# Safari77/rupphash

Hardware: AMD Instinct MI355X
Metric: pdq_hashes_per_sec_512x512_rgb (higher is better)
Workload: dtype f32

## Files before the change

### rupphash_amd/csrc/pdq_fused512.hip

```cpp
#include "pdq_tail.hpp"
#include "rph_internal.h"

namespace {

typedef _Float16 h2 __attribute__((ext_vector_type(2)));
typedef _Float16 h8 __attribute__((ext_vector_type(8)));

template <int SW_, int CH_ = 3, bool PARK_ = true>
struct Geo {
    static constexpr int SW = SW_;
    static constexpr int CH = CH_;
    static constexpr int NSTRIP = 512 / SW;
    static constexpr int CL = SW / 8;
    static constexpr int NG = 64 / CL;
    static constexpr int NH = 64 / (NG * 8);
    static constexpr int NOCT = SW / 8;
    static constexpr int TILE_PITCH = SW * 2 + 16;
    static constexpr int TILE_BYTES = 64 * TILE_PITCH;
    static constexpr int OFF_TILE = 0;
    static constexpr int OFF_XCHG = NH == 2 ? 32 * TILE_PITCH : 0;
    static constexpr int OFF_STATE = TILE_BYTES;
    static constexpr int OFF_EDGE = OFF_STATE + 7168;
#ifndef RPH_PARK_CHAINS
#define RPH_PARK_CHAINS 1
#endif
    static constexpr bool PARK = RPH_PARK_CHAINS && PARK_ && SW == 64;
    static constexpr int OFF_PARK_C = OFF_EDGE + 1536;
    static constexpr int OFF_PARK_E = OFF_PARK_C + (PARK ? 9 * 64 * 4 : 0);
    static constexpr int LDS_BYTES = OFF_PARK_E + (PARK ? 9 * 6 * 4 : 0);
    static constexpr int WAVES_PER_SIMD = 2;
    static constexpr bool AHEAD = SW == 64;
    static_assert(64 * 33 * 4 <= TILE_BYTES, "sample transpose buffer must fit in the dead V tile");
    static_assert((NG - 1) * 7 * CL * 16 <= (NH == 2 ? 32 : 64) * TILE_PITCH, "exchange area must fit");
    static_assert(rph::TAIL_LDS_FLOATS * 4 <= TILE_BYTES, "tail scratch must fit in the dead V tile");
};
constexpr int SAMP_PITCH = 33;

struct Px8 {
    uint32_t d[6];
};
struct __attribute__((packed, aligned(4))) U3 {
    uint32_t x, y, z;
};

struct __attribute__((packed, aligned(4))) U2 {
    uint32_t x, y;
};
template <int CH = 3>
__device__ __forceinline__ Px8 load_px8(const uint8_t *p)
{
    Px8 r;
    if (CH == 1) {
        const U2 a = *reinterpret_cast<const U2 *>(p);
        r.d[0] = a.x; r.d[1] = a.y; r.d[2] = r.d[3] = r.d[4] = r.d[5] = 0;
        return r;
    }
    const U3 a = *reinterpret_cast<const U3 *>(p);
    const U3 b = *reinterpret_cast<const U3 *>(p + 12);
    r.d[0] = a.x; r.d[1] = a.y; r.d[2] = a.z; r.d[3] = b.x; r.d[4] = b.y; r.d[5] = b.z;
    return r;
}

template <int P>
__device__ __forceinline__ float luma_px(const Px8 &v)
{
    constexpr int B = 3 * P;
    const float r = (float)((v.d[B >> 2] >> (8 * (B & 3))) & 0xFFu);
    const float g = (float)((v.d[(B + 1) >> 2] >> (8 * ((B + 1) & 3))) & 0xFFu);
    const float b = (float)((v.d[(B + 2) >> 2] >> (8 * ((B + 2) & 3))) & 0xFFu);
    const float num = __builtin_fmaf(299.0f, r, __builtin_fmaf(587.0f, g, __builtin_fmaf(114.0f, b, 500.0f)));
    return __builtin_truncf(num * 0.001f);
}

template <int CH = 3>
__device__ __forceinline__ void luma8(const Px8 &v, float (&l)[8])
{
    if (CH == 1) {
#pragma unroll
        for (int i = 0; i < 8; i++) l[i] = (float)((v.d[i >> 2] >> (8 * (i & 3))) & 0xFFu);
        return;
    }
    l[0] = luma_px<0>(v); l[1] = luma_px<1>(v); l[2] = luma_px<2>(v); l[3] = luma_px<3>(v);
    l[4] = luma_px<4>(v); l[5] = luma_px<5>(v); l[6] = luma_px<6>(v); l[7] = luma_px<7>(v);
}

constexpr uint32_t BIASED_ZERO = 0x64006400u;
struct Row8 {
    h2 q[4];
};
__device__ __forceinline__ h2 h2_bits(uint32_t u) { return __builtin_bit_cast(h2, u); }
__device__ __forceinline__ h2 byte_pair_lo(uint32_t d) { return h2_bits(__builtin_amdgcn_perm(0x64646464u, d, 0x04010400u)); }
__device__ __forceinline__ h2 byte_pair_hi(uint32_t d) { return h2_bits(__builtin_amdgcn_perm(0x64646464u, d, 0x04030402u)); }

__device__ __forceinline__ float dot2_from_zero(h2 a, h2 k, uint32_t after)
{
    float r;
    asm volatile("v_dot2_f32_f16 %0, %1, %2, 0" : "=v"(r) : "v"(__builtin_bit_cast(uint32_t, a)), "s"(__builtin_bit_cast(uint32_t, k)), "v"(after));
    return r;
}

struct Pairs12 {
    h2 P[12];
};
__device__ __forceinline__ Pairs12 byte_pairs(const Px8 &v)
{
    Pairs12 r;
#pragma unroll
    for (int i = 0; i < 6; i++) {
        r.P[2 * i] = byte_pair_lo(v.d[i]);
        r.P[2 * i + 1] = byte_pair_hi(v.d[i]);
    }
    return r;
}
__device__ __forceinline__ Row8 luma_row(const Pairs12 &pr, bool zero, uint32_t &order)
{
    const h2 *P = pr.P;
    const h2 k_rg = h2{(_Float16)299.0f, (_Float16)587.0f};
    const h2 k_b0 = h2{(_Float16)114.0f, (_Float16)0.0f};
    const h2 k_0r = h2{(_Float16)0.0f, (_Float16)299.0f};
    const h2 k_gb = h2{(_Float16)587.0f, (_Float16)114.0f};
    float vhalf;
    asm("v_mov_b32 %0, 0.5" : "=v"(vhalf));
    h2 packed[4];
#pragma unroll
    for (int pp = 0; pp < 4; pp++) {
        const float n0 = __builtin_amdgcn_fdot2(P[3 * pp], k_rg, dot2_from_zero(P[3 * pp + 1], k_b0, order), false);
        const float n1 = __builtin_amdgcn_fdot2(P[3 * pp + 1], k_0r, dot2_from_zero(P[3 * pp + 2], k_gb, order), false);
        const float y0 = __builtin_fmaf(n0, 0.001f, vhalf), y1 = __builtin_fmaf(n1, 0.001f, vhalf);
        packed[pp] = __builtin_bit_cast(h2, __builtin_amdgcn_cvt_pkrtz(y0, y1));
    }
    order = __builtin_bit_cast(uint32_t, packed[3]);
    Row8 r;
#pragma unroll
    for (int i = 0; i < 4; i++) {
        r.q[i] = packed[i];
        if (zero) r.q[i] = h2_bits(BIASED_ZERO);
    }
    return r;
}
__device__ __forceinline__ Row8 luma_row_gray(const Px8 &v, bool zero, uint32_t &order)
{
    Row8 r;
    r.q[0] = byte_pair_lo(v.d[0]);
    r.q[1] = byte_pair_hi(v.d[0]);
    r.q[2] = byte_pair_lo(v.d[1]);
    r.q[3] = byte_pair_hi(v.d[1]);
#pragma unroll
    for (int i = 0; i < 4; i++)
        if (zero) r.q[i] = h2_bits(BIASED_ZERO);
    order = __builtin_bit_cast(uint32_t, r.q[3]);
    return r;
}
template <int CH = 3>
__device__ __forceinline__ Row8 pack_row(const Px8 &v, bool zero, uint32_t &order)
{
    if (CH == 1) return luma_row_gray(v, zero, order);
    return luma_row(byte_pairs(v), zero, order);
}
__device__ __forceinline__ uint4 row_bits(const Row8 &r)
{
    uint4 u;
    u.x = __builtin_bit_cast(uint32_t, r.q[0]);
    u.y = __builtin_bit_cast(uint32_t, r.q[1]);
    u.z = __builtin_bit_cast(uint32_t, r.q[2]);
    u.w = __builtin_bit_cast(uint32_t, r.q[3]);
    return u;
}
__device__ __forceinline__ Row8 bits_row(const uint4 &u)
{
    Row8 r;
    r.q[0] = __builtin_bit_cast(h2, u.x);
    r.q[1] = __builtin_bit_cast(h2, u.y);
    r.q[2] = __builtin_bit_cast(h2, u.z);
    r.q[3] = __builtin_bit_cast(h2, u.w);
    return r;
}

__device__ __forceinline__ float div_small(float N, float d, float dinv)
{
    const float q0 = N * dinv;
    const float r = __builtin_fmaf(-q0, d, N);
    return __builtin_fmaf(r, dinv, q0);
}

__device__ __forceinline__ void wave_lds_fence() { asm volatile("" ::: "memory"); }

struct Wave {
    uint8_t *lds;
    const uint8_t *img;
    size_t row_stride;
    uint32_t rs32;
    int lane;
    float hs, sum, ring[8];
    uint4 pv;
    float row_d8, row_dinv8;
    float smp[32];
    float smp_last;
    float csum, cring[8];
    float ecs, ering[8];
    float bnew[8];
    rph::TailAcc tail;
    bool want_quality;
};

template <class G>
__device__ __forceinline__ int half_row(int b, int h, int g, int k) { return 64 * b + 4 + (G::NG * 8) * h + 8 * g + k; }

template <class G>
__device__ __forceinline__ void half_offsets(const Wave &w, int b, int s, int h, uint32_t &off0, uint32_t &off_max)
{
    const int c = w.lane & (G::CL - 1), g = w.lane / G::CL;
    const uint32_t col = (uint32_t)(G::SW * s + 8 * c) * (uint32_t)G::CH;
    off0 = (uint32_t)half_row<G>(b, h, g, 0) * w.rs32 + col;
    off_max = 511u * w.rs32 + col;
}
template <int CH>
__device__ __forceinline__ Px8 load_px8_at(const Wave &w, uint32_t off) { return load_px8<CH>(w.img + off); }

template <class G>
__device__ __forceinline__ void half_issue(const Wave &w, int b, int s, int h, Px8 (&pre)[8])
{
    uint32_t off, off_max;
    half_offsets<G>(w, b, s, h, off, off_max);
#pragma unroll
    for (int k = 0; k < 8; k++) {
        pre[k] = load_px8_at<G::CH>(w, off);
        off = off + w.rs32;
        off = off < off_max ? off : off_max;
    }
}

template <class G, bool LAST_BAND>
__device__ __forceinline__ void half_luma(const Wave &w, int b, int h, Px8 (&pre)[8], Row8 (&L)[8], bool has_next, int nb, int ns, int nh)
{
    const int g = w.lane / G::CL;
    uint32_t off, off_max;
    half_offsets<G>(w, nb, ns, nh, off, off_max);
    uint32_t order = 0;
#pragma unroll
    for (int k = 0; k < 8; k++) {
        if (G::CH == 1) {
            const Px8 cur = pre[k];
            if (has_next) pre[k] = load_px8_at<1>(w, off);
            off = off + w.rs32;
            off = off < off_max ? off : off_max;
            L[k] = luma_row_gray(cur, LAST_BAND && (half_row<G>(b, h, g, k) >= 512), order);
            continue;
        }
        const Pairs12 pr = byte_pairs(pre[k]);
        if (has_next) pre[k] = load_px8_at<3>(w, off);
        off = off + w.rs32;
        off = off < off_max ? off : off_max;
        L[k] = luma_row(pr, LAST_BAND && (half_row<G>(b, h, g, k) >= 512), order);
    }
}

template <class G>
__device__ __forceinline__ void half_build(Wave &w, int s, int h, const Row8 (&L)[8])
{
    const int c = w.lane & (G::CL - 1), g = w.lane / G::CL;
    uint8_t *tile = w.lds + G::OFF_TILE;
    uint8_t *xchg = w.lds + G::OFF_XCHG;
    uint8_t *state = w.lds + G::OFF_STATE + (G::SW * s + 8 * c) * 2;

    if (g < G::NG - 1) {
        uint8_t *x = xchg + ((g * 7) * G::CL + c) * 16;
#pragma unroll
        for (int k = 1; k < 8; k++) *reinterpret_cast<uint4 *>(x + (k - 1) * (G::CL * 16)) = row_bits(L[k]);
    }
    wave_lds_fence();
    Row8 hist[7];
    {
        const uint8_t *hp = (g == 0) ? state : xchg + (((g - 1) * 7) * G::CL + c) * 16;
        const int stride = (g == 0) ? 1024 : G::CL * 16;
#pragma unroll
        for (int j = 0; j < 7; j++) hist[j] = bits_row(*reinterpret_cast<const uint4 *>(hp + j * stride));
    }
    wave_lds_fence();
    if (g == G::NG - 1) {
#pragma unroll
        for (int k = 1; k < 8; k++) *reinterpret_cast<uint4 *>(state + (k - 1) * 1024) = row_bits(L[k]);
    }
    const int row0 = (G::NG * 8) * h + 8 * g;
    Row8 v;
#pragma unroll
    for (int i = 0; i < 4; i++) {
        const h2 two_bias = h2{(_Float16)2048.0f, (_Float16)2048.0f};
        h2 a = hist[0].q[i] + (hist[1].q[i] - two_bias);
        h2 bb = hist[2].q[i] + (hist[3].q[i] - two_bias);
        h2 cc = hist[4].q[i] + (hist[5].q[i] - two_bias);
        h2 dd = hist[6].q[i] + (L[0].q[i] - two_bias);
        v.q[i] = (a + bb) + (cc + dd);
    }
    *reinterpret_cast<uint4 *>(tile + (row0 + 0) * G::TILE_PITCH + 16 * c) = row_bits(v);
#pragma unroll
    for (int m = 1; m < 8; m++) {
#pragma unroll
        for (int i = 0; i < 4; i++) v.q[i] = (v.q[i] - hist[m - 1].q[i]) + L[m].q[i];
        *reinterpret_cast<uint4 *>(tile + (row0 + m) * G::TILE_PITCH + 16 * c) = row_bits(v);
    }
    wave_lds_fence();
}

__device__ __forceinline__ uint32_t h2_diff(uint32_t cur, uint32_t prev)
{
    return __builtin_bit_cast(uint32_t, __builtin_bit_cast(h2, cur) - __builtin_bit_cast(h2, prev));
}
template <int HI>
__device__ __forceinline__ float hs_step(float hs, uint32_t packed)
{
    float r;
    if (HI)
        asm("v_fma_mix_f32 %0, %1, 1.0, %2 op_sel:[1,0,0] op_sel_hi:[1,0,0]" : "=v"(r) : "v"(packed), "v"(hs));
    else
        asm("v_fma_mix_f32 %0, %1, 1.0, %2 op_sel:[0,0,0] op_sel_hi:[1,0,0]" : "=v"(r) : "v"(packed), "v"(hs));
    return r;
}
template <int HI>
__device__ __forceinline__ float hs_sub(float hs, uint32_t packed)
{
    float r;
    if (HI)
        asm("v_fma_mix_f32 %0, %1, -1.0, %2 op_sel:[1,0,0] op_sel_hi:[1,0,0]" : "=v"(r) : "v"(packed), "v"(hs));
    else
        asm("v_fma_mix_f32 %0, %1, -1.0, %2 op_sel:[0,0,0] op_sel_hi:[1,0,0]" : "=v"(r) : "v"(packed), "v"(hs));
    return r;
}

template <int E>
__device__ __forceinline__ void row_step(Wave &w, float in2)
{
    constexpr int slot = (E + 4) & 7;
    w.sum = w.sum + in2;
    w.sum = w.sum - w.ring[slot];
    w.ring[slot] = in2;
}

template <bool EDGE_ROWS>
__device__ __forceinline__ float pass1_value(const Wave &w, float hs)
{
    if (EDGE_ROWS) return div_small(hs, w.row_d8, w.row_dinv8);
    return hs;
}

template <class G, bool EDGE_ROWS, bool FIRST, bool LAST>
__device__ __forceinline__ void scan_strip(Wave &w)
{
    const int r = w.lane;
    const uint8_t *tp = w.lds + G::OFF_TILE + r * G::TILE_PITCH;
    const float *edge = reinterpret_cast<const float *>(w.lds + G::OFF_EDGE);
    float fresh[G::NOCT];
#pragma unroll
    for (int q = 0; q < G::NOCT; q++) {
        const uint4 cur = *reinterpret_cast<const uint4 *>(tp + 16 * q);
        const uint32_t dq[4] = {h2_diff(cur.x, w.pv.x), h2_diff(cur.y, w.pv.y), h2_diff(cur.z, w.pv.z), h2_diff(cur.w, w.pv.w)};
        const bool first_octet = FIRST && q == 0;
        float e0 = 0.f, e1 = 0.f, e2 = 0.f;
        if (first_octet) {
            e0 = edge[0 * 64 + r];
            e1 = edge[1 * 64 + r];
            e2 = edge[2 * 64 + r];
        }
#define RPH_STEP(E)                                                              \
    {                                                                            \
        w.hs = hs_step<(E) & 1>(w.hs, dq[(E) >> 1]);                             \
        float in2 = pass1_value<EDGE_ROWS>(w, w.hs);                             \
        if (first_octet && (E) == 4) in2 = e0;                                   \
        if (first_octet && (E) == 5) in2 = e1;                                   \
        if (first_octet && (E) == 6) in2 = e2;                                   \
        if (!(first_octet && (E) < 4)) row_step<E>(w, in2);  \
    }
        RPH_STEP(0) RPH_STEP(1) RPH_STEP(2) RPH_STEP(3) RPH_STEP(4)
        fresh[q] = w.sum * 0.125f;
        RPH_STEP(5) RPH_STEP(6) RPH_STEP(7)
#undef RPH_STEP
        w.pv = cur;
    }
    if (LAST) {
        const float e3 = edge[3 * 64 + r], e4 = edge[4 * 64 + r], e5 = edge[5 * 64 + r];
        w.hs = hs_sub<0>(w.hs, w.pv.x); row_step<0>(w, e3);
        w.hs = hs_sub<1>(w.hs, w.pv.x); row_step<1>(w, e4);
        w.hs = hs_sub<0>(w.hs, w.pv.y); row_step<2>(w, e5);
        w.hs = hs_sub<1>(w.hs, w.pv.y);
        {
            const float in511 = (EDGE_ROWS ? div_small(w.hs, w.row_d8, w.row_dinv8) : w.hs) * 2.0f;
            row_step<3>(w, in511);
        }
        w.sum = w.sum - w.ring[0];
        w.smp_last = w.sum / 7.0f;
    }
#pragma unroll
    for (int i = 0; i < 32 - G::NOCT; i++) w.smp[i] = w.smp[i + G::NOCT];
#pragma unroll
    for (int q = 0; q < G::NOCT; q++) w.smp[32 - G::NOCT + q] = fresh[q];
}

__device__ __forceinline__ void scan_reset(Wave &w, int b)
{
    w.hs = 0.f;
    w.sum = 0.f;
#pragma unroll
    for (int i = 0; i < 8; i++) w.ring[i] = 0.f;
    w.pv = make_uint4(0, 0, 0, 0);
    const int y = 64 * b + w.lane;
    const int lo = y - 3 < 0 ? 0 : y - 3, hi = y + 4 > 511 ? 511 : y + 4;
    const float d = (float)(hi - lo + 1);
    w.row_d8 = d * 0.125f;
    w.row_dinv8 = (1.0f / d) * 8.0f;
}

template <class G, bool NEXT_EDGE = false>
__device__ __forceinline__ void col_pass(Wave &w, int b, bool second_half, Px8 (*epx)[2] = nullptr)
{
    float *tb = reinterpret_cast<float *>(w.lds + G::OFF_TILE);
#pragma unroll
    for (int t = 0; t < 32; t++) tb[w.lane * SAMP_PITCH + t] = w.smp[t];
    tb[w.lane * SAMP_PITCH + 32] = w.smp_last;
    if (NEXT_EDGE) edge_band_issue<G>(w, b + 1, *epx);
    wave_lds_fence();
    const bool active = second_half ? (w.lane >= 31) : (w.lane < 31);
    if (active) {
        float *park = reinterpret_cast<float *>(w.lds + G::OFF_PARK_C) + w.lane;
        if (G::PARK) {
            w.csum = park[0];
#pragma unroll
            for (int e = 0; e < 8; e++) w.cring[e] = park[64 * (e + 1)];
        }
        const float *samp = tb + (second_half ? w.lane - 31 : w.lane + 1);
#pragma unroll
        for (int u = 0; u < 8; u++) {
            float in[8];
#pragma unroll
            for (int e = 0; e < 8; e++) in[e] = samp[(8 * u + e) * SAMP_PITCH];
#pragma unroll
            for (int e = 0; e < 8; e++) {
                w.csum = w.csum + in[e];
                w.csum = w.csum - w.cring[e];
                w.cring[e] = in[e];
                if (e == 0) w.bnew[u] = w.csum * (0.125f * 0.015625f);
            }
        }
        if (G::PARK) {
            park[0] = w.csum;
#pragma unroll
            for (int e = 0; e < 8; e++) park[64 * (e + 1)] = w.cring[e];
        }
    }
    wave_lds_fence();
}

template <int CH>
__device__ __forceinline__ void edge_issue(const Wave &w, int y, Px8 (&e)[2])
{
    const int yc = y > 511 ? 511 : y;
    e[0] = load_px8<CH>(w.img + (size_t)yc * w.row_stride);
    e[1] = load_px8<CH>(w.img + (size_t)yc * w.row_stride + 504 * CH);
}
__device__ __forceinline__ void edge_values(const float (&l)[8], const float (&r)[8], bool live, float (&rv)[6])
{
    const float r0 = (((l[0] + l[1]) + l[2]) + l[3]) + l[4];
    const float r1 = r0 + l[5];
    const float r2 = r1 + l[6];
    const float q510 = (((r[3] + r[4]) + r[5]) + r[6]) + r[7];
    const float q509 = q510 + r[2];
    const float q508 = q509 + r[1];
    rv[0] = div_small(r0 * 64.0f, 5.0f, 1.0f / 5.0f);
    rv[1] = div_small(r1 * 64.0f, 6.0f, 1.0f / 6.0f);
    rv[2] = div_small(r2 * 64.0f, 7.0f, 1.0f / 7.0f);
    rv[3] = div_small(q508 * 64.0f, 7.0f, 1.0f / 7.0f);
    rv[4] = div_small(q509 * 64.0f, 6.0f, 1.0f / 6.0f);
    rv[5] = div_small(q510 * 64.0f, 5.0f, 1.0f / 5.0f);
    if (!live) {
#pragma unroll
        for (int k = 0; k < 6; k++) rv[k] = 0.f;
    }
}
template <int CH>
__device__ __forceinline__ void edge_compute(const Px8 (&e)[2], bool live, float (&rv)[6])
{
    float l[8], r[8];
    luma8<CH>(e[0], l);
    luma8<CH>(e[1], r);
    edge_values(l, r, live, rv);
}
template <int CH>
__device__ __forceinline__ void edge_rowvals(const Wave &w, int y, bool live, float (&rv)[6])
{
    Px8 e[2];
    edge_issue<CH>(w, y, e);
    edge_compute<CH>(e, live, rv);
}

template <class G>
__device__ __forceinline__ void edge_prologue(Wave &w)
{
    float *edge = reinterpret_cast<float *>(w.lds + G::OFF_EDGE);
    float rv[6];
    {
        const uint8_t *row = w.lds + G::OFF_STATE + (3 + (w.lane & 3)) * 1024;
        const h8 hl = *reinterpret_cast<const h8 *>(row), hr = *reinterpret_cast<const h8 *>(row + 504 * 2);
        float l[8], r[8];
#pragma unroll
        for (int i = 0; i < 8; i++) {
            l[i] = (float)hl[i] - 1024.0f;
            r[i] = (float)hr[i] - 1024.0f;
        }
        edge_values(l, r, true, rv);
    }
    if (w.lane < 4) {
#pragma unroll
        for (int k = 0; k < 6; k++) edge[k * 64 + w.lane] = rv[k];
    }
    wave_lds_fence();
    w.ecs = 0.f;
#pragma unroll
    for (int i = 0; i < 8; i++) w.ering[i] = 0.f;
    if (w.lane < 6) {
#pragma unroll
        for (int t = 0; t < 4; t++) {
            const float v = edge[w.lane * 64 + t];
            w.ecs = w.ecs + v;
            w.ering[t] = v;
        }
        if (G::PARK) {
            float *park = reinterpret_cast<float *>(w.lds + G::OFF_PARK_E) + w.lane;
            park[0] = w.ecs;
#pragma unroll
            for (int i = 0; i < 8; i++) park[6 * (i + 1)] = w.ering[i];
        }
    }
    wave_lds_fence();
}

template <class G>
__device__ __forceinline__ void edge_band_issue(const Wave &w, int b, Px8 (&epx)[2]) { edge_issue<G::CH>(w, 64 * b + 4 + w.lane, epx); }

template <class G, int KIND>
__device__ __forceinline__ void edge_band(Wave &w, int b, const Px8 (&epx)[2])
{
    float *edge = reinterpret_cast<float *>(w.lds + G::OFF_EDGE);
    {
        float rv[6];
        const int y = 64 * b + 4 + w.lane;
        edge_compute<G::CH>(epx, y < 512, rv);
#pragma unroll
        for (int k = 0; k < 6; k++) edge[k * 64 + w.lane] = rv[k];
    }
    wave_lds_fence();
    if (w.lane < 6) {
        float *mine = edge + w.lane * 64;
        float *park = reinterpret_cast<float *>(w.lds + G::OFF_PARK_E) + w.lane;
        if (G::PARK) {
            w.ecs = park[0];
#pragma unroll
            for (int i = 0; i < 8; i++) w.ering[i] = park[6 * (i + 1)];
        }
#pragma unroll 1
        for (int u = 0; u < 8; u++) {
            float in[8], out[8];
#pragma unroll
            for (int e = 0; e < 8; e++) in[e] = mine[8 * u + e];
#pragma unroll
            for (int e = 0; e < 8; e++) {
                constexpr int dummy = 0;
                (void)dummy;
                const int slot = (e + 4) & 7;
                const bool add = !(KIND == 2 && u == 7 && e >= 4);
                if (add) w.ecs = w.ecs + in[e];
                w.ecs = w.ecs - w.ering[slot];
                w.ering[slot] = in[e];
                float o;
                if (KIND == 0 && u == 0 && e < 3)
                    o = w.ecs / (float)(5 + e);
                else if (KIND == 2 && u == 7 && e >= 4)
                    o = w.ecs / (float)(11 - e);
                else
                    o = w.ecs * 0.125f;
                out[e] = o;
            }
#pragma unroll
            for (int e = 0; e < 8; e++) mine[8 * u + e] = out[e];
        }
        if (G::PARK) {
            park[0] = w.ecs;
#pragma unroll
            for (int i = 0; i < 8; i++) park[6 * (i + 1)] = w.ering[i];
        }
    }
    wave_lds_fence();
}

template <class G>
__device__ __forceinline__ void store_samples(const Wave &w, float *band_samples, bool second_half)
{
    float *p = band_samples + (second_half ? 32 * 64 : 0) + w.lane;
    asm volatile("" : "+v"(p));
#pragma unroll
    for (int t = 0; t < 32; t++) p[t * 64] = w.smp[t];
    if (second_half) p[32 * 64] = w.smp_last;
}

template <class G, int KIND, bool LL = false>
__device__ __forceinline__ void do_band(Wave &w, int b, Px8 (&pre)[8], float *samples, Px8 (&epx)[2])
{
    constexpr bool EDGE_ROWS = KIND != 1;
    if (!LL) {
        if (!G::AHEAD) edge_band_issue<G>(w, b, epx);
        edge_band<G, KIND>(w, b, epx);
    }
    scan_reset(w, b);
#pragma unroll 1
    for (int s = 0; s < G::NSTRIP; s++) {
#pragma unroll 1
        for (int h = 0; h < G::NH; h++) {
            Row8 L[8];
            int nb = b, ns = s, nh = h + 1;
            if (nh == G::NH) {
                nh = 0;
                ns = s + 1;
                if (ns == G::NSTRIP) {
                    ns = 0;
                    nb = b + 1;
                }
            }
            half_luma<G, KIND == 2>(w, b, h, pre, L, LL ? nb == b : nb < 8, nb, ns, nh);
            half_build<G>(w, s, h, L);
        }
        if (s == 0)
            scan_strip<G, EDGE_ROWS, true, false>(w);
        else if (s == G::NSTRIP - 1)
            scan_strip<G, EDGE_ROWS, false, true>(w);
        else
            scan_strip<G, EDGE_ROWS, false, false>(w);
        wave_lds_fence();
        if (LL) {
            if (s == G::NSTRIP / 2 - 1) store_samples<G>(w, samples, false);
            if (s == G::NSTRIP - 1) store_samples<G>(w, samples, true);
        } else {
            if (s == G::NSTRIP / 2 - 1) col_pass<G>(w, b, false);
            if (!G::AHEAD && s == G::NSTRIP - 1) col_pass<G>(w, b, true);
        }
        wave_lds_fence();
    }
    if (LL) return;
    if (G::AHEAD) {
        col_pass<G, KIND != 2>(w, b, true, &epx);
        wave_lds_fence();
    }
#pragma unroll
    for (int u = 0; u < 8; u++)
        if (KIND != 0 || u > 0) rph::tail_row(w.tail, w.bnew[u], 8 * b + u - 1, w.lane, w.want_quality);
}

template <class G>
__global__ void __launch_bounds__(64, G::WAVES_PER_SIMD) pdq_fused512_kernel(const uint8_t *__restrict__ px, uint32_t n, size_t row_stride,
                                                          size_t image_stride, uint8_t *hash, float *quality, float *coeffs,
                                                          uint8_t *dihedral, uint8_t *valid)
{
    __shared__ __attribute__((aligned(16))) uint8_t lds[G::LDS_BYTES];
    const uint32_t img = blockIdx.x;
    Wave w;
    w.lds = lds;
    w.img = px + (size_t)img * image_stride;
    w.row_stride = row_stride;
    w.rs32 = (uint32_t)row_stride;
    w.lane = threadIdx.x;
    Px8 head[4], epx[2], pre[8];
    if (G::AHEAD) {
#pragma unroll
        for (int row = 0; row < 4; row++) head[row] = load_px8<G::CH>(w.img + (size_t)row * row_stride + (size_t)(8 * w.lane) * G::CH);
        edge_band_issue<G>(w, 0, epx);
    }
    half_issue<G>(w, 0, 0, 0, pre);
    wave_lds_fence();
    w.csum = 0.f;
    w.smp_last = 0.f;
#pragma unroll
    for (int i = 0; i < 32; i++) w.smp[i] = 0.f;
#pragma unroll
    for (int i = 0; i < 8; i++) w.cring[i] = 0.f;
    if (G::PARK) {
#pragma unroll
        for (int i = 0; i < 9; i++) reinterpret_cast<float *>(lds + G::OFF_PARK_C)[64 * i + w.lane] = 0.f;
    }
    rph::tail_init(w.tail);
    w.want_quality = quality != nullptr;
#pragma unroll
    for (int u = 0; u < 8; u++) w.bnew[u] = 0.f;

    {
        for (int j = 0; j < 3; j++)
            for (int t = w.lane; t < 64; t += 64) *reinterpret_cast<uint4 *>(lds + G::OFF_STATE + j * 1024 + t * 16) = make_uint4(BIASED_ZERO, BIASED_ZERO, BIASED_ZERO, BIASED_ZERO);
        uint32_t order = 0;
        if (G::AHEAD) {
#pragma unroll
            for (int row = 0; row < 4; row++)
                *reinterpret_cast<uint4 *>(lds + G::OFF_STATE + (3 + row) * 1024 + (8 * w.lane) * 2) = row_bits(pack_row<G::CH>(head[row], false, order));
        } else {
#pragma unroll 1
            for (int it = 0; it < 4; it++) {
                const int slot = it * 64 + w.lane;
                const int chunk = slot & 63, row = slot >> 6;
                const Px8 p = load_px8<G::CH>(w.img + (size_t)row * row_stride + (size_t)(8 * chunk) * G::CH);
                *reinterpret_cast<uint4 *>(lds + G::OFF_STATE + (3 + row) * 1024 + (8 * chunk) * 2) = row_bits(pack_row<G::CH>(p, false, order));
            }
        }
    }
    wave_lds_fence();
    edge_prologue<G>(w);

    do_band<G, 0>(w, 0, pre, nullptr, epx);
#pragma unroll 1
    for (int b = 1; b < 7; b++) do_band<G, 1>(w, b, pre, nullptr, epx);
    do_band<G, 2>(w, 7, pre, nullptr, epx);

    if (G::PARK) {
        w.csum = reinterpret_cast<const float *>(lds + G::OFF_PARK_C)[w.lane];
        w.cring[0] = reinterpret_cast<const float *>(lds + G::OFF_PARK_C)[64 + w.lane];
    }
    w.csum = w.csum - w.cring[0];
    rph::tail_row(w.tail, (w.csum / 7.0f) * 0.015625f, 63, w.lane, w.want_quality);

    __syncthreads();
    rph::tail_finish(w.tail, reinterpret_cast<float *>(lds), w.lane, hash + (size_t)img * 32, quality ? quality + img : nullptr,
                  coeffs ? coeffs + (size_t)img * 256 : nullptr, dihedral ? dihedral + (size_t)img * 256 : nullptr);
    if (valid && w.lane == 0) valid[img] = 1;
}

constexpr int LL_SAMPLE_FLOATS = 8 * 65 * 64;
constexpr int LL_EDGE_PITCH = 520;

template <class G, int KIND>
__device__ __forceinline__ void ll_band(Wave &w, int b, float *samples)
{
    Px8 pre[8];
    half_issue<G>(w, b, 0, 0, pre);
    Px8 none[2];
    do_band<G, KIND, true>(w, b, pre, samples, none);
}

template <class G>
__global__ void __launch_bounds__(512, 2) pdq_fused512_ll_kernel(const uint8_t *__restrict__ px, uint32_t n, size_t row_stride, size_t image_stride,
                                                                 float *__restrict__ sample_scratch, uint8_t *hash, float *quality, float *coeffs,
                                                                 uint8_t *dihedral, uint8_t *valid)
{
    static_assert(G::NH == 1, "the low-latency kernel is built on the 64-px strip geometry");
    __shared__ __attribute__((aligned(16))) uint8_t lds[8 * G::LDS_BYTES + 6 * LL_EDGE_PITCH * 4];
    const uint32_t img = blockIdx.x;
    const int band = __builtin_amdgcn_readfirstlane(threadIdx.x >> 6);
    Wave w;
    w.lds = lds + band * G::LDS_BYTES;
    w.img = px + (size_t)img * image_stride;
    w.row_stride = row_stride;
    w.rs32 = (uint32_t)row_stride;
    w.lane = threadIdx.x & 63;
    w.smp_last = 0.f;
#pragma unroll
    for (int i = 0; i < 32; i++) w.smp[i] = 0.f;
    w.want_quality = quality != nullptr;
    float *edge_all = reinterpret_cast<float *>(lds + 8 * G::LDS_BYTES);
    float *samples = sample_scratch + (size_t)img * LL_SAMPLE_FLOATS;

    {
        float rv[6];
        edge_rowvals<G::CH>(w, 64 * band + w.lane, true, rv);
#pragma unroll
        for (int k = 0; k < 6; k++) edge_all[k * LL_EDGE_PITCH + 64 * band + w.lane] = rv[k];
        if (band == 7 && w.lane < 8) {
#pragma unroll
            for (int k = 0; k < 6; k++) edge_all[k * LL_EDGE_PITCH + 512 + w.lane] = 0.f;
        }
    }
    {
        uint32_t order = 0;
#pragma unroll 1
        for (int it = 0; it < 7; it++) {
            const int row = 64 * band - 3 + it;
            uint4 bits = make_uint4(BIASED_ZERO, BIASED_ZERO, BIASED_ZERO, BIASED_ZERO);
            if (row >= 0) bits = row_bits(pack_row<G::CH>(load_px8<G::CH>(w.img + (size_t)row * row_stride + (size_t)(8 * w.lane) * G::CH), false, order));
            *reinterpret_cast<uint4 *>(w.lds + G::OFF_STATE + it * 1024 + (8 * w.lane) * 2) = bits;
        }
    }
    __syncthreads();
    if (w.lane < 6) {
        const float *in = edge_all + w.lane * LL_EDGE_PITCH;
        float *mine = reinterpret_cast<float *>(w.lds + G::OFF_EDGE) + w.lane * 64;
        float ecs = 0.f, ering[8];
#pragma unroll
        for (int t = 0; t < 8; t++) ering[t] = 0.f;
#pragma unroll
        for (int t = 0; t < 4; t++) {
            ecs = ecs + in[t];
            ering[t] = in[t];
        }
#pragma unroll 1
        for (int bb = 0; bb < band; bb++)
#pragma unroll 1
            for (int u = 0; u < 8; u++) {
                float v[8];
#pragma unroll
                for (int e = 0; e < 8; e++) v[e] = in[64 * bb + 4 + 8 * u + e];
#pragma unroll
                for (int e = 0; e < 8; e++) {
                    ecs = ecs + v[e];
                    ecs = ecs - ering[(e + 4) & 7];
                    ering[(e + 4) & 7] = v[e];
                }
            }
#pragma unroll 1
        for (int u = 0; u < 8; u++) {
            float v[8], out[8];
#pragma unroll
            for (int e = 0; e < 8; e++) v[e] = in[64 * band + 4 + 8 * u + e];
#pragma unroll
            for (int e = 0; e < 8; e++) {
                const bool past_end = band == 7 && u == 7 && e >= 4;
                if (!past_end) ecs = ecs + v[e];
                ecs = ecs - ering[(e + 4) & 7];
                ering[(e + 4) & 7] = v[e];
                float o = ecs * 0.125f;
                if (band == 0 && u == 0 && e < 3) o = ecs / (float)(5 + e);
                if (past_end) o = ecs / (float)(11 - e);
                out[e] = o;
            }
#pragma unroll
            for (int e = 0; e < 8; e++) mine[8 * u + e] = out[e];
        }
    }
    wave_lds_fence();

    float *band_samples = samples + (size_t)band * (65 * 64);
    if (band == 0)
        ll_band<G, 0>(w, 0, band_samples);
    else if (band == 7)
        ll_band<G, 2>(w, 7, band_samples);
    else
        ll_band<G, 1>(w, band, band_samples);
    __syncthreads();
    if (band != 0) return;

    w.csum = 0.f;
#pragma unroll
    for (int i = 0; i < 8; i++) w.cring[i] = 0.f;
    rph::tail_init(w.tail);
    const float *col = samples + (size_t)(w.lane + 1) * 64;
#pragma unroll 1
    for (int bb = 0; bb < 8; bb++) {
        const float *cb = col + (size_t)bb * (65 * 64);
#pragma unroll 1
        for (int u = 0; u < 8; u++) {
            const float4 lo = *reinterpret_cast<const float4 *>(cb + 8 * u), hi = *reinterpret_cast<const float4 *>(cb + 8 * u + 4);
            const float in[8] = {lo.x, lo.y, lo.z, lo.w, hi.x, hi.y, hi.z, hi.w};
            float bnew = 0.f;
#pragma unroll
            for (int e = 0; e < 8; e++) {
                w.csum = w.csum + in[e];
                w.csum = w.csum - w.cring[e];
                w.cring[e] = in[e];
                if (e == 0) bnew = w.csum * (0.125f * 0.015625f);
            }
            if (bb != 0 || u != 0) rph::tail_row(w.tail, bnew, 8 * bb + u - 1, w.lane, w.want_quality);
        }
    }
    w.csum = w.csum - w.cring[0];
    rph::tail_row(w.tail, (w.csum / 7.0f) * 0.015625f, 63, w.lane, w.want_quality);
    wave_lds_fence();
    rph::tail_finish(w.tail, reinterpret_cast<float *>(w.lds), w.lane, hash + (size_t)img * 32, quality ? quality + img : nullptr,
                     coeffs ? coeffs + (size_t)img * 256 : nullptr, dihedral ? dihedral + (size_t)img * 256 : nullptr);
    if (valid && w.lane == 0) valid[img] = 1;
}

}

int rph_launch_pdq_fused512_ll(rph_ctx *ctx, const uint8_t *d_px, uint32_t n, size_t row_stride, size_t image_stride, uint8_t *d_hash,
                               float *d_quality, float *d_coeffs, uint8_t *d_dihedral, uint8_t *d_valid, hipStream_t stream)
{
    if (n == 0) return RPH_OK;
    const uint32_t chunk = n < 256 ? n : 256;
    const size_t need = (size_t)chunk * LL_SAMPLE_FLOATS * sizeof(float);
    if (ctx->ll_scratch.size() > 256 && ctx->ll_scratch.find(stream) == ctx->ll_scratch.end()) {
        RPH_HIP_CHECK(hipDeviceSynchronize());
        ctx->ll_scratch.clear();
    }
    DevBuf &sc = ctx->ll_scratch[stream];
    RPH_TRY(sc.reserve(need, stream));
    for (uint32_t first = 0; first < n; first += chunk) {
        const uint32_t m = (n - first) < chunk ? (n - first) : chunk;
        hipLaunchKernelGGL((pdq_fused512_ll_kernel<Geo<64, 3, false>>), dim3(m), dim3(512), 0, stream, d_px + (size_t)first * image_stride, m, row_stride, image_stride,
                           sc.as<float>(), d_hash + (size_t)first * 32, d_quality ? d_quality + first : nullptr, d_coeffs ? d_coeffs + (size_t)first * 256 : nullptr,
                           d_dihedral ? d_dihedral + (size_t)first * 256 : nullptr, d_valid ? d_valid + first : nullptr);
        RPH_HIP_CHECK(hipGetLastError());
    }
    return RPH_OK;
}

int rph_launch_pdq_fused512(rph_ctx *ctx, const uint8_t *d_px, uint32_t n, size_t row_stride, size_t image_stride,
                            uint8_t *d_hash, float *d_quality, float *d_coeffs, uint8_t *d_dihedral, uint8_t *d_valid,
                            hipStream_t stream, uint32_t channels)
{
    if (n == 0) return RPH_OK;
    if (channels == 1) {
        hipLaunchKernelGGL((pdq_fused512_kernel<Geo<64, 1>>), dim3(n), dim3(64), 0, stream, d_px, n, row_stride, image_stride, d_hash, d_quality, d_coeffs, d_dihedral,
                           d_valid);
        RPH_HIP_CHECK(hipGetLastError());
        return RPH_OK;
    }
    if (ctx->pdq_kernel == 3 || ((ctx->pdq_kernel == 4 || ctx->pdq_kernel == 6) && n < 768))
        return rph_launch_pdq_fused512_ll(ctx, d_px, n, row_stride, image_stride, d_hash, d_quality, d_coeffs, d_dihedral, d_valid, stream);
    if (ctx->pdq_kernel == 2)
        hipLaunchKernelGGL(pdq_fused512_kernel<Geo<128>>, dim3(n), dim3(64), 0, stream, d_px, n, row_stride, image_stride, d_hash,
                           d_quality, d_coeffs, d_dihedral, d_valid);
    else
        hipLaunchKernelGGL(pdq_fused512_kernel<Geo<64>>, dim3(n), dim3(64), 0, stream, d_px, n, row_stride, image_stride, d_hash,
                           d_quality, d_coeffs, d_dihedral, d_valid);
    RPH_HIP_CHECK(hipGetLastError());
    return RPH_OK;
}
```

### rupphash_amd/csrc/pdq_tail.hpp

```cpp
#pragma once
#include <hip/hip_runtime.h>
#include <stdint.h>

#include "dct_table.h"

namespace rph {

struct DctT {
    uint32_t v[1024];
};
constexpr DctT make_dct_t()
{
    constexpr uint32_t src[1024] = RPH_DCT_TABLE_INIT;
    DctT t{};
    for (int k = 0; k < 64; k++)
        for (int i = 0; i < 16; i++) t.v[k * 16 + i] = src[i * 64 + k];
    return t;
}
__constant__ DctT c_dct_t = make_dct_t();

constexpr int TAIL_LDS_FLOATS = 16 * 65 + 256;

__device__ __forceinline__ void tail_fence() { asm volatile("" ::: "memory"); }

__device__ __forceinline__ uint32_t total_key(float f)
{
    const uint32_t b = __float_as_uint(f);
    return b ^ ((b >> 31) ? 0xFFFFFFFFu : 0x80000000u);
}
__device__ __forceinline__ float key_to_float(uint32_t k)
{
    return __uint_as_float((k & 0x80000000u) ? (k ^ 0x80000000u) : ~k);
}

__device__ __forceinline__ uint32_t select_rank127(const uint32_t (&key)[4])
{
    uint32_t prefix = 0, mask = 0;
    int k = 127;
#pragma unroll 1
    for (int bit = 31; bit >= 0; --bit) {
        const uint32_t b = 1u << bit;
        int cnt = 0;
#pragma unroll
        for (int m = 0; m < 4; m++) cnt += __popcll(__ballot(((key[m] & mask) == prefix) && !(key[m] & b)));
        if (k >= cnt) {
            k -= cnt;
            prefix |= b;
        }
        mask |= b;
    }
    return prefix;
}

__device__ __forceinline__ void emit_hash(const float (&v)[4], float median, uint8_t *out32, int lane)
{
    unsigned long long bal[4];
#pragma unroll
    for (int m = 0; m < 4; m++) bal[m] = __ballot(v[m] > median);
    if (lane < 32) {
        const int r = (31 - lane) >> 1;
        const unsigned long long bb = (r >> 2) == 0 ? bal[0] : ((r >> 2) == 1 ? bal[1] : ((r >> 2) == 2 ? bal[2] : bal[3]));
        const uint32_t row = (uint32_t)(bb >> (16 * (r & 3))) & 0xFFFFu;
        out32[lane] = (uint8_t)((lane & 1) ? (row & 0xFFu) : (row >> 8));
    }
}

__device__ __forceinline__ float median_of(const float (&v)[4])
{
    uint32_t key[4];
#pragma unroll
    for (int m = 0; m < 4; m++) key[m] = total_key(v[m]);
    return key_to_float(select_rank127(key));
}

__device__ __forceinline__ void hashes_from_coeffs(const float (&c)[4], float *lds_c, int lane, uint8_t *hash32,
                                                   uint8_t *dihedral)
{
    const float med0 = median_of(c);
    if (hash32) emit_hash(c, med0, hash32, lane);
    if (!dihedral) return;

    const int cc = lane & 15;
    tail_fence();
#pragma unroll
    for (int m = 0; m < 4; m++) lds_c[lane + 64 * m] = c[m];
    tail_fence();
    float t[4];
#pragma unroll
    for (int m = 0; m < 4; m++) t[m] = lds_c[16 * cc + ((lane >> 4) + 4 * m)];

    const bool c_even = (cc & 1) == 0;
    float nr[4], nc[4], nb[4];
    float tnr[4], tnc[4], tnb[4];
#pragma unroll
    for (int m = 0; m < 4; m++) {
        const bool r_even = ((((lane >> 4) + 4 * m)) & 1) == 0;
        nr[m] = r_even ? -c[m] : c[m];
        nc[m] = c_even ? -c[m] : c[m];
        nb[m] = (r_even != c_even) ? -c[m] : c[m];
        tnr[m] = c_even ? -t[m] : t[m];
        tnc[m] = r_even ? -t[m] : t[m];
        tnb[m] = (r_even != c_even) ? -t[m] : t[m];
    }
    const float med_nr = median_of(nr), med_nc = median_of(nc), med_nb = median_of(nb);
    emit_hash(c, med0, dihedral + 0 * 32, lane);
    emit_hash(tnr, med_nr, dihedral + 1 * 32, lane);
    emit_hash(nb, med_nb, dihedral + 2 * 32, lane);
    emit_hash(tnc, med_nc, dihedral + 3 * 32, lane);
    emit_hash(nc, med_nc, dihedral + 4 * 32, lane);
    emit_hash(nr, med_nr, dihedral + 5 * 32, lane);
    emit_hash(t, med0, dihedral + 6 * 32, lane);
    emit_hash(tnb, med_nb, dihedral + 7 * 32, lane);
}

struct TailAcc {
    float t[16];
    float qsum;
    float prev;
};

__device__ __forceinline__ void tail_init(TailAcc &a)
{
#pragma unroll
    for (int i = 0; i < 16; i++) a.t[i] = 0.0f;
    a.qsum = 0.0f;
    a.prev = 0.0f;
}

__device__ __forceinline__ void tail_row(TailAcc &a, float brow, int k, int lane, bool want_quality)
{
#pragma unroll
    for (int i = 0; i < 16; i++) {
        const float p = __uint_as_float(c_dct_t.v[k * 16 + i]) * brow;
        a.t[i] = a.t[i] + p;
    }
    if (want_quality) {
        const float right = __shfl_down(brow, 1);
        const float gh = truncf(fabsf(((brow - right) * 100.0f) / 255.0f));
        const float gv = truncf(fabsf(((a.prev - brow) * 100.0f) / 255.0f));
        a.qsum += (lane < 63) ? gh : 0.0f;
        a.qsum += (k > 0) ? gv : 0.0f;
    }
    a.prev = brow;
}

__device__ __forceinline__ void tail_row_left(TailAcc &a, float brow, float left, bool has_left, int k, bool want_quality)
{
#pragma unroll
    for (int i = 0; i < 16; i++) {
        const float p = __uint_as_float(c_dct_t.v[k * 16 + i]) * brow;
        a.t[i] = a.t[i] + p;
    }
    if (want_quality) {
        const float gh = truncf(fabsf(((left - brow) * 100.0f) / 255.0f));
        const float gv = truncf(fabsf(((a.prev - brow) * 100.0f) / 255.0f));
        a.qsum += has_left ? gh : 0.0f;
        a.qsum += (k > 0) ? gv : 0.0f;
    }
    a.prev = brow;
}

__device__ __forceinline__ void tail_finish(TailAcc &a, float *lds, int lane, uint8_t *hash32, float *quality, float *coeffs,
                                            uint8_t *dihedral)
{
    if (quality) {
        float acc = a.qsum;
#pragma unroll
        for (int off = 32; off > 0; off >>= 1) acc += __shfl_xor(acc, off);
        const float q = acc / 90.0f;
        if (lane == 0) *quality = q > 1.0f ? 1.0f : q;
    }
    float *lds_t = lds;
    float *lds_c = lds + 16 * 65;
    tail_fence();
#pragma unroll
    for (int i = 0; i < 16; i++) lds_t[i * 65 + lane] = a.t[i];
    tail_fence();

    float c[4] = {0.0f, 0.0f, 0.0f, 0.0f};
    const int jj = lane & 15, i0 = lane >> 4;
#pragma unroll 8
    for (int k = 0; k < 64; k++) {
        const float dj = __uint_as_float(c_dct_t.v[k * 16 + jj]);
#pragma unroll
        for (int m = 0; m < 4; m++) {
            const float p = lds_t[(i0 + 4 * m) * 65 + k] * dj;
            c[m] = c[m] + p;
        }
    }
    if (coeffs) {
#pragma unroll
        for (int m = 0; m < 4; m++) coeffs[lane + 64 * m] = c[m];
    }
    hashes_from_coeffs(c, lds_c, lane, hash32, dihedral);
}

__device__ __forceinline__ void pdq_tail(const float (&b)[64], float *lds, int lane, uint8_t *hash32, float *quality,
                                         float *coeffs, uint8_t *dihedral)
{
    TailAcc a;
    tail_init(a);
#pragma unroll
    for (int k = 0; k < 64; k++) tail_row(a, b[k], k, lane, quality != nullptr);
    tail_finish(a, lds, lane, hash32, quality, coeffs, dihedral);
}

}
```

Baseline: 6.915 million.

## Pair edge-row divisions, drop per-row clamp, and early-exit median radix select

```diff
diff --git a/rupphash_amd/csrc/pdq_fused512.hip b/rupphash_amd/csrc/pdq_fused512.hip
--- a/rupphash_amd/csrc/pdq_fused512.hip
+++ b/rupphash_amd/csrc/pdq_fused512.hip
@@ -30,6 +30,7 @@
     static constexpr int LDS_BYTES = OFF_PARK_E + (PARK ? 9 * 6 * 4 : 0);
     static constexpr int WAVES_PER_SIMD = 2;
     static constexpr bool AHEAD = SW == 64;
+    static constexpr bool PAIR_QUOT = SW == 64;
     static_assert(64 * 33 * 4 <= TILE_BYTES, "sample transpose buffer must fit in the dead V tile");
     static_assert((NG - 1) * 7 * CL * 16 <= (NH == 2 ? 32 : 64) * TILE_PITCH, "exchange area must fit");
     static_assert(rph::TAIL_LDS_FLOATS * 4 <= TILE_BYTES, "tail scratch must fit in the dead V tile");
@@ -181,6 +182,16 @@
     const float q0 = N * dinv;
     const float r = __builtin_fmaf(-q0, d, N);
     return __builtin_fmaf(r, dinv, q0);
+}
+
+typedef float f2 __attribute__((ext_vector_type(2)));
+__device__ __forceinline__ f2 div_small2(f2 N, f2 d, f2 dinv)
+{
+    f2 q0;
+    q0.x = N.x * dinv.x;
+    q0.y = N.y * dinv.y;
+    const f2 r = __builtin_elementwise_fma(-q0, d, N);
+    return __builtin_elementwise_fma(r, dinv, q0);
 }
 
 __device__ __forceinline__ void wave_lds_fence() { asm volatile("" ::: "memory"); }
@@ -204,29 +215,36 @@
 };
 
 template <class G>
-__device__ __forceinline__ int half_row(int b, int h, int g, int k) { return 64 * b + 4 + (G::NG * 8) * h + 8 * g + k; }
+constexpr __device__ __forceinline__ int half_row(int b, int h, int g, int k) { return 64 * b + 4 + (G::NG * 8) * h + 8 * g + k; }
 
 template <class G>
-__device__ __forceinline__ void half_offsets(const Wave &w, int b, int s, int h, uint32_t &off0, uint32_t &off_max)
+__device__ __forceinline__ uint32_t half_offset(const Wave &w, int b, int s, int h)
 {
     const int c = w.lane & (G::CL - 1), g = w.lane / G::CL;
     const uint32_t col = (uint32_t)(G::SW * s + 8 * c) * (uint32_t)G::CH;
-    off0 = (uint32_t)half_row<G>(b, h, g, 0) * w.rs32 + col;
-    off_max = 511u * w.rs32 + col;
+    return (uint32_t)half_row<G>(b, h, g, 0) * w.rs32 + col;
+}
+template <class G>
+__device__ __forceinline__ uint32_t half_row_fold(const Wave &w, int b, int h)
+{
+    static_assert(half_row<G>(7, G::NH - 1, G::NG - 1, 4) == 512 && half_row<G>(7, G::NH - 1, G::NG - 2, 7) < 512, "rows >= 512: last lane group, rows 4..7");
+    const int g = w.lane / G::CL;
+    return (b == 7 && h == G::NH - 1 && g == G::NG - 1) ? 4u * w.rs32 : 0u;
 }
 template <int CH>
-__device__ __forceinline__ Px8 load_px8_at(const Wave &w, uint32_t off) { return load_px8<CH>(w.img + off); }
+__device__ __forceinline__ Px8 load_px8_row(const Wave &w, int k, uint32_t off)
+{
+    return load_px8<CH>(w.img + (size_t)k * w.row_stride + off);
+}
 
 template <class G>
 __device__ __forceinline__ void half_issue(const Wave &w, int b, int s, int h, Px8 (&pre)[8])
 {
-    uint32_t off, off_max;
-    half_offsets<G>(w, b, s, h, off, off_max);
+    uint32_t off = half_offset<G>(w, b, s, h);
 #pragma unroll
     for (int k = 0; k < 8; k++) {
-        pre[k] = load_px8_at<G::CH>(w, off);
-        off = off + w.rs32;
-        off = off < off_max ? off : off_max;
+        if (k == 4) off -= half_row_fold<G>(w, b, h);
+        pre[k] = load_px8_row<G::CH>(w, k, off);
     }
 }
 
@@ -234,24 +252,21 @@
 __device__ __forceinline__ void half_luma(const Wave &w, int b, int h, Px8 (&pre)[8], Row8 (&L)[8], bool has_next, int nb, int ns, int nh)
 {
     const int g = w.lane / G::CL;
-    uint32_t off, off_max;
-    half_offsets<G>(w, nb, ns, nh, off, off_max);
+    uint32_t off = half_offset<G>(w, nb, ns, nh);
     uint32_t order = 0;
 #pragma unroll
     for (int k = 0; k < 8; k++) {
+        if (k == 4) off -= half_row_fold<G>(w, nb, nh);
+        const bool zero = LAST_BAND && (half_row<G>(b, h, g, k) >= 512);
         if (G::CH == 1) {
             const Px8 cur = pre[k];
-            if (has_next) pre[k] = load_px8_at<1>(w, off);
-            off = off + w.rs32;
-            off = off < off_max ? off : off_max;
-            L[k] = luma_row_gray(cur, LAST_BAND && (half_row<G>(b, h, g, k) >= 512), order);
+            if (has_next) pre[k] = load_px8_row<1>(w, k, off);
+            L[k] = luma_row_gray(cur, zero, order);
             continue;
         }
         const Pairs12 pr = byte_pairs(pre[k]);
-        if (has_next) pre[k] = load_px8_at<3>(w, off);
-        off = off + w.rs32;
-        off = off < off_max ? off : off_max;
-        L[k] = luma_row(pr, LAST_BAND && (half_row<G>(b, h, g, k) >= 512), order);
+        if (has_next) pre[k] = load_px8_row<3>(w, k, off);
+        L[k] = luma_row(pr, zero, order);
     }
 }
 
@@ -350,6 +365,7 @@
     const uint8_t *tp = w.lds + G::OFF_TILE + r * G::TILE_PITCH;
     const float *edge = reinterpret_cast<const float *>(w.lds + G::OFF_EDGE);
     float fresh[G::NOCT];
+    const f2 d2 = {w.row_d8, w.row_d8}, dinv2 = {w.row_dinv8, w.row_dinv8};
 #pragma unroll
     for (int q = 0; q < G::NOCT; q++) {
         const uint4 cur = *reinterpret_cast<const uint4 *>(tp + 16 * q);
@@ -370,9 +386,25 @@
         if (first_octet && (E) == 6) in2 = e2;                                   \
         if (!(first_octet && (E) < 4)) row_step<E>(w, in2);  \
     }
-        RPH_STEP(0) RPH_STEP(1) RPH_STEP(2) RPH_STEP(3) RPH_STEP(4)
-        fresh[q] = w.sum * 0.125f;
-        RPH_STEP(5) RPH_STEP(6) RPH_STEP(7)
+#define RPH_PAIR(E, BETWEEN)                                                     \
+    {                                                                            \
+        f2 hp;                                                                   \
+        hp.x = hs_step<0>(w.hs, dq[(E) >> 1]);                                   \
+        hp.y = hs_step<1>(hp.x, dq[(E) >> 1]);                                   \
+        w.hs = hp.y;                                                             \
+        const f2 in2 = div_small2(hp, d2, dinv2);                                \
+        row_step<(E)>(w, in2.x);                                                 \
+        BETWEEN;                                                                 \
+        row_step<(E) + 1>(w, in2.y);                                             \
+    }
+        if (G::PAIR_QUOT && EDGE_ROWS && !first_octet) {
+            RPH_PAIR(0, (void)0) RPH_PAIR(2, (void)0) RPH_PAIR(4, fresh[q] = w.sum * 0.125f) RPH_PAIR(6, (void)0)
+        } else {
+            RPH_STEP(0) RPH_STEP(1) RPH_STEP(2) RPH_STEP(3) RPH_STEP(4)
+            fresh[q] = w.sum * 0.125f;
+            RPH_STEP(5) RPH_STEP(6) RPH_STEP(7)
+        }
+#undef RPH_PAIR
 #undef RPH_STEP
         w.pv = cur;
     }
diff --git a/rupphash_amd/csrc/pdq_tail.hpp b/rupphash_amd/csrc/pdq_tail.hpp
--- a/rupphash_amd/csrc/pdq_tail.hpp
+++ b/rupphash_amd/csrc/pdq_tail.hpp
@@ -36,20 +36,31 @@
 __device__ __forceinline__ uint32_t select_rank127(const uint32_t (&key)[4])
 {
     uint32_t prefix = 0, mask = 0;
-    int k = 127;
+    int k = 127, cand = 256;
 #pragma unroll 1
     for (int bit = 31; bit >= 0; --bit) {
         const uint32_t b = 1u << bit;
+        mask |= b;
         int cnt = 0;
 #pragma unroll
-        for (int m = 0; m < 4; m++) cnt += __popcll(__ballot(((key[m] & mask) == prefix) && !(key[m] & b)));
+        for (int m = 0; m < 4; m++) cnt += __popcll(__ballot((key[m] & mask) == prefix));
         if (k >= cnt) {
             k -= cnt;
+            cand -= cnt;
             prefix |= b;
+        } else {
+            cand = cnt;
         }
-        mask |= b;
-    }
-    return prefix;
+        if (cand == 1) break;
+    }
+    if (cand != 1) return prefix;
+    uint32_t found = prefix;
+#pragma unroll
+    for (int m = 0; m < 4; m++) {
+        const unsigned long long hit = __ballot((key[m] & mask) == prefix);
+        if (hit) found = (uint32_t)__builtin_amdgcn_readlane((int)key[m], __ffsll(hit) - 1);
+    }
+    return found;
 }
 
 __device__ __forceinline__ void emit_hash(const float (&v)[4], float median, uint8_t *out32, int lane)
```

New measurement: 7.008 million (median of 6 runs). +1.3%, better.
